# iresearch-toolkit/iresearch

Measured on AMD Instinct MI355X. Metric: queries/sec BM25 top-1000, OR-8-terms, 10M-doc Zipfian index @1/2/4/8 GPU, higher is better.
Workload: dtype u32+f32

## Files before the change

### include/irs_hip.h

```cpp
#ifndef IRS_HIP_H
#define IRS_HIP_H

#include <stddef.h>
#include <stdint.h>

#ifdef __cplusplus
extern "C" {
#endif

#define IRS_HIP_ABI_VERSION 12
#define IRS_HIP_BLOCK_SIZE 128u
#define IRS_HIP_MAX_TERMS 16u
#define IRS_HIP_MAX_K 4096u
#define IRS_HIP_MAX_PHRASE_TERMS 8u
#define IRS_HIP_MAX_PHRASE_ENTRIES 16u
#define IRS_HIP_MAX_EXCLUDED 16u
#define IRS_HIP_NO_TERM 0xFFFFFFFFu
#define IRS_HIP_POS_OFFSETS 1u
#define IRS_HIP_POS_PAYLOADS 2u
#define IRS_HIP_NORM2 0u
#define IRS_HIP_NORM_LEGACY 1u
#define IRS_HIP_WAND_NONE 0u
#define IRS_HIP_WAND_DIV_NORM 1u
#define IRS_HIP_WAND_MAX_FREQ 2u
// ... 214 lines not shown
int irs_hip_device_download(int32_t device, void* h_dst, const void* d_src, uint64_t bytes);
int irs_hip_device_sync(int32_t device, void* stream);
int irs_hip_device_trim(int32_t device);

int irs_hip_device_set_stream_cache(int32_t device, uint64_t bytes);
typedef struct irs_hip_stream_cache_stats {
  uint64_t bytes_held;
  uint64_t budget;
  uint64_t streams;
  uint64_t hits;
  uint64_t misses;
  uint64_t evictions;
} irs_hip_stream_cache_stats;
int irs_hip_device_stream_cache_stats(int32_t device, irs_hip_stream_cache_stats* out);
int irs_hip_batch_stream_counts(irs_hip_batch* batch, uint32_t* distinct, uint32_t* decoded);
int irs_hip_batch_image_counts(irs_hip_batch* batch, uint32_t* distinct, uint32_t* built);
int irs_hip_batch_rescore_paths(irs_hip_batch* batch, uint32_t paths[3]);
int irs_hip_device_image_count(int32_t device, uint64_t* images);
int irs_hip_join_bound_rule(int32_t kind, float norm_const, float norm_length, uint32_t tf_bound,
                            uint16_t* u, float* scale, float* slack, uint32_t* tile_docs);

typedef struct irs_hip_comm irs_hip_comm;
#define IRS_HIP_COMM_ID_BYTES 128u
int irs_hip_comm_unique_id(uint8_t id[IRS_HIP_COMM_ID_BYTES]);
int irs_hip_comm_init_rank(int32_t device, const uint8_t id[IRS_HIP_COMM_ID_BYTES], int32_t n_ranks,
                           int32_t rank, irs_hip_comm** out);
void irs_hip_comm_destroy(irs_hip_comm* comm);
int irs_hip_comm_library(char* buf, size_t cap);
int irs_hip_topk_allgather(irs_hip_comm* comm, const void* d_send, void* d_recv,
                           uint64_t bytes_per_rank, void* stream);
// ... 12 lines not shown
```

### iresearch_amd/_lib.py

```python
from __future__ import annotations

import ctypes as C

import numpy as np

from . import _build

OK, EINVAL, ECORRUPT, ENOMEM, EHIP, EOVERFLOW, EUNSUPPORTED, EPEER = 0, -1, -2, -3, -4, -5, -6, -7
LAYOUT_SCALAR, LAYOUT_SIMD4 = 0, 1
OP_OR, OP_AND, OP_MINMATCH, OP_PHRASE = 0, 1, 2, 3
SCORE_BM25, SCORE_BM15, SCORE_BM1, SCORE_TFIDF, SCORE_TFIDF_NORM = 0, 1, 2, 3, 4
EXCLUDE = 0x100
PHRASE_ALT = 0x200
GROUP_ALT = PHRASE_ALT
PHRASE_REQUIRED = 0x400
NO_TERM = 0xFFFFFFFF
NO_DOC_SET = 0xFFFFFFFF
PATH_AUTO, PATH_ITEMS, PATH_JOINED = 0, 1, 2
WAND_NONE, WAND_DIV_NORM, WAND_MAX_FREQ, WAND_MIN_NORM = 0, 1, 2, 3
MAX_TERMS, MAX_K, MAX_PHRASE_TERMS, MAX_EXCLUDED = 16, 4096, 8, 16
MAX_PHRASE_ENTRIES = 16
K_PLAN, K_PILOT, K_SCORE, K_SELECT, K_COUNT = 0, 1, 2, 3, 4
KERNEL_NAMES = ("k_plan", "k_pilot", "k_score", "k_select")
KERNEL_NAMES_JOINED = ("k_join", "k_join_pilot", "k_join_score", "k_select")
# ... 51 lines not shown
    "irs_hip_batch_set_async", "irs_hip_batch_set_paired_tiles", "irs_hip_batch_paired_tiles",
    "irs_hip_batch_set_comm",
    "irs_hip_term_blockmax",
    "irs_hip_segment_wand_source",
    "irs_hip_batch_touched", "irs_hip_batch_unit_mask",
    "irs_hip_batch_match_sets", "irs_hip_batch_match_sets_to_device",
    "irs_hip_batch_set_doc_sets", "irs_hip_batch_set_doc_sets_host", "irs_hip_batch_doc_set_stats",
    "irs_hip_comm_unique_id", "irs_hip_comm_init_rank", "irs_hip_comm_destroy",
    "irs_hip_comm_library",
    "irs_hip_topk_allgather", "irs_hip_device_alloc", "irs_hip_device_free",
    "irs_hip_device_upload", "irs_hip_device_download", "irs_hip_device_sync",
    "irs_hip_device_trim",
    "irs_hip_device_set_stream_cache", "irs_hip_device_stream_cache_stats",
    "irs_hip_batch_stream_counts",
    "irs_hip_batch_image_counts", "irs_hip_device_image_count", "irs_hip_join_bound_rule",
    "irs_hip_batch_rescore_paths",
)


def bind(L: C.CDLL) -> C.CDLL:
    vp, u32, u64, i32 = C.c_void_p, C.c_uint32, C.c_uint64, C.c_int32
    P = C.POINTER
    L.irs_hip_abi_version.argtypes, L.irs_hip_abi_version.restype = [], u32
    L.irs_hip_strerror.argtypes, L.irs_hip_strerror.restype = [C.c_int], C.c_char_p
    L.irs_hip_device_arch.argtypes, L.irs_hip_device_arch.restype = [i32, C.c_char_p, C.c_size_t], C.c_int
    L.irs_hip_segment_open.argtypes = [P(SegmentDesc), P(vp)]
    L.irs_hip_segment_open.restype = C.c_int
    L.irs_hip_segment_close.argtypes, L.irs_hip_segment_close.restype = [vp], None
    L.irs_hip_segment_device_bytes.argtypes = [vp]
    L.irs_hip_segment_device_bytes.restype = u64
    L.irs_hip_segment_live_docs.argtypes = [vp]
# ... 75 lines not shown
    L.irs_hip_topk_allgather.restype = C.c_int
    L.irs_hip_device_trim.argtypes, L.irs_hip_device_trim.restype = [i32], C.c_int
    L.irs_hip_device_set_stream_cache.argtypes = [i32, u64]
    L.irs_hip_device_set_stream_cache.restype = C.c_int
    L.irs_hip_device_stream_cache_stats.argtypes = [i32, P(StreamCacheStats)]
    L.irs_hip_device_stream_cache_stats.restype = C.c_int
    L.irs_hip_batch_stream_counts.argtypes = [vp, P(u32), P(u32)]
    L.irs_hip_batch_stream_counts.restype = C.c_int
    L.irs_hip_batch_image_counts.argtypes = [vp, P(u32), P(u32)]
    L.irs_hip_batch_image_counts.restype = C.c_int
    L.irs_hip_device_image_count.argtypes, L.irs_hip_device_image_count.restype = [i32, P(u64)], C.c_int
    L.irs_hip_batch_rescore_paths.argtypes, L.irs_hip_batch_rescore_paths.restype = [vp, P(u32)], C.c_int
    L.irs_hip_join_bound_rule.argtypes = [i32, C.c_float, C.c_float, u32, P(C.c_uint16), P(C.c_float),
                                          P(C.c_float), P(u32)]
    L.irs_hip_join_bound_rule.restype = C.c_int
    return L


_lib = None


def lib() -> C.CDLL:
    global _lib
    if _lib is None:
        try:
            import torch
        except ImportError:
            pass
        _lib = bind(C.CDLL(str(_build.build_hip())))
    return _lib
# ... 6 lines not shown
```

### iresearch_amd/csrc/irs_hip.hip

```cpp
#include "irs_hip.h"

#include <algorithm>
#include <atomic>
#include <chrono>
#include <cmath>
#include <condition_variable>
#include <cstdlib>
#include <cstring>
#include <deque>
#include <functional>
#include <map>
#include <memory>
#include <mutex>
#include <new>
#include <thread>
#include <tuple>
#include <type_traits>
#include <unordered_map>
#include <unordered_set>
#include <vector>

#include "gpu_rt.h"
#include "kernels.h"
#include "phrase.h"
// ... 1698 lines not shown
  return guarded([&] {
    if (slack) *slack = kJoinBoundSlack;
    if (tile_docs) *tile_docs = kJoinBoundTile;
    if (!table_kind(kind)) return int(IRS_HIP_EUNSUPPORTED);
    const float sup = join_bound_sup(kind, norm_const, norm_length, tf_bound);
    if (!(sup > 0.f)) return int(IRS_HIP_EUNSUPPORTED);
    const float U = join_bound_scale(sup);
    if (scale) *scale = U;
    if (u)
      for (uint32_t tf = 0; tf < 256u; ++tf)
        for (uint32_t n = 0; n < 256u; ++n)
          u[tf * 256u + n] = uint16_t(join_bound_u(kind, norm_const, norm_length, U, tf, n));
    return int(IRS_HIP_OK);
  });
}
int irs_hip_device_sync(int32_t device, void* stream) {
  return guarded([&] {
    if (!rt::set_device(device)) return int(IRS_HIP_EHIP);
    return int(rt::sync(static_cast<rt::stream_t>(stream)) ? IRS_HIP_OK : IRS_HIP_EHIP);
  });
}
int irs_hip_comm_unique_id(uint8_t id[IRS_HIP_COMM_ID_BYTES]) {
  return guarded([&]() -> int {
    if (!id) return IRS_HIP_EINVAL;
    return rt::comm::unique_id(id) ? IRS_HIP_OK : IRS_HIP_EHIP;
  });
}
int irs_hip_comm_init_rank(int32_t device, const uint8_t id[IRS_HIP_COMM_ID_BYTES], int32_t n_ranks,
                           int32_t rank, irs_hip_comm** out) {
  return guarded([&] { return comm_init_rank_impl(device, id, n_ranks, rank, out); });
// ... 100 lines not shown
```

### iresearch_amd/csrc/join.h

```cpp
#pragma once
#include "score.h"

namespace irs_hip {

constexpr uint32_t kJoinTile = 12288;
constexpr uint32_t kJoinTfMax = 255;
constexpr uint32_t kJoinBlocks = 64;
constexpr uint32_t kJoinChunkTiles = 64;
constexpr uint32_t kJoinChunkPlain = 32;
constexpr uint32_t kJoinCands = 256;
constexpr uint32_t kJoinSlack = 1024;
constexpr uint32_t kJoinQueues = 8;
constexpr uint32_t kAblShift = 0;
constexpr uint32_t kAblCount = 0;
constexpr uint32_t kAblEpi = 0;
constexpr uint32_t kAblNoAdd = 0;
constexpr uint32_t kAblNoTab = 0;
constexpr uint32_t kAblWait = 0;
constexpr uint32_t kAblNoBar = 0;
constexpr uint32_t kJoinCountMask = 15u;
constexpr uint32_t kJoinCountTerms = 15u;
constexpr float kJoinCountRound = 8.f;

enum : uint32_t {
// ... 251 lines not shown
  }
  if (!(sup > 0.f) || !(sup <= 3.0e38f)) return 0.f;
  if (!sqrt_kind(kind) && sup < kJoinBoundSupMin) return 0.f;
  return sup;
}
__host__ __device__ inline float join_bound_scale(float sup) { return (65535.f - 64.f) / sup; }
__host__ __device__ inline uint32_t join_bound_u(int32_t kind, float nc, float nl, float U,
                                                 uint32_t tf, uint32_t norm) {
  const float tref = table_entry(kind, nc, nl, tf ? tf : 1u, norm);
  const float tb = tref + tref * (1.f / 524288.f) + (sqrt_kind(kind) ? 0.f : (1.f / 1048576.f));
  const float r = tb * U + 1.25f;
  const uint32_t u = r >= 65535.f ? 65535u : static_cast<uint32_t>(r);
  return u;
}

struct alignas(16) BoundWg {
  uint64_t src, src_bounds;
  uint64_t dst, dst_bounds;
  uint32_t first;
  uint32_t n;
  uint32_t n_src_tiles, n_dst_tiles;
  int32_t kind;
  float nc, nl;
  float U;
};
static_assert(sizeof(BoundWg) == 64, "BoundWg");

__global__ void __launch_bounds__(kThreads)
k_join_bound(const BoundWg* wgs) {
  const BoundWg W = wgs[blockIdx.x];
  const uint32_t* src = reinterpret_cast<const uint32_t*>(W.src);
  const uint32_t* sb = reinterpret_cast<const uint32_t*>(W.src_bounds);
  uint32_t* dst = reinterpret_cast<uint32_t*>(W.dst);
  uint32_t* db = reinterpret_cast<uint32_t*>(W.dst_bounds);
  if (!W.n) {
    for (uint32_t u = threadIdx.x; u <= W.n_dst_tiles; u += blockDim.x) db[u] = 0u;
    return;
  }
  auto tile_of = [&](uint32_t i, uint32_t lo) {
    uint32_t hi = W.n_src_tiles;
    while (hi - lo > 1u) {
      const uint32_t mid = (lo + hi) >> 1;
      if (sb[mid] <= i) lo = mid; else hi = mid;
    }
    return lo;
  };
  uint32_t t = 0;
  const uint32_t end = W.first + kJoinBoundPerWg < W.n ? W.first + kJoinBoundPerWg : W.n;
  for (uint32_t i = W.first + threadIdx.x; i < end; i += blockDim.x) {
    t = tile_of(i, t);
    const uint32_t e = src[i];
    const uint32_t doc = t * kJoinTile + (e >> 18);
    const uint32_t bt = doc / kJoinBoundTile;
    const uint32_t off = doc - bt * kJoinBoundTile;
    const uint32_t u = join_bound_u(W.kind, W.nc, W.nl, W.U, join_tf(e), (e >> 2) & 255u);
    dst[i] = (off << 18) | u;
    int32_t tp = -1;
    if (i) {
      const uint32_t pt = sb[t] < i ? t : tile_of(i - 1u, 0u);
      tp = int32_t((pt * kJoinTile + (src[i - 1u] >> 18)) / kJoinBoundTile);
    }
    for (int32_t v = tp + 1; v <= int32_t(bt); ++v) db[v] = i;
    if (i + 1u == W.n)
      for (uint32_t v = bt + 1u; v <= W.n_dst_tiles; ++v) db[v] = W.n;
  }
}


struct JoinOff {
  static constexpr uint32_t acc = 0;
  static constexpr uint32_t dummy = 4u * kJoinTile;
  static constexpr uint32_t qts = dummy + 256u;
  static constexpr uint32_t jts = qts + uint32_t(sizeof(DevQTerm)) * kMaxTerms;
  static constexpr uint32_t rng = jts + uint32_t(sizeof(JoinTerm)) * kMaxTerms;
  static constexpr uint32_t cum = rng + 4u * (kJoinChunkTiles + 1u) * kMaxTerms;
  static constexpr uint32_t sig = cum + 4u * kJoinChunkTiles * kMaxTerms;
  static constexpr uint32_t cand = sig + 4u * 2u * 16u;
  static constexpr uint32_t vars = cand + 8u * 2u * kJoinCands;
  static constexpr uint32_t caches = vars + 64u;
// ... 25 lines not shown
};

struct JoinLane {
  uint32_t ent_lo, ent_hi;
  float cs;
  uint32_t mode;
};

enum : int { kJTable = 0, kJRcp = 1, kJSqrt = 2 };
__device__ __forceinline__ int join_form(uint32_t mode) {
  return !(mode & kJoinGeneral) ? kJTable : ((mode & kJoinSqrt) ? kJSqrt : kJRcp);
}
__device__ __forceinline__ uint32_t join_dummy(unsigned lane) {
  return (JoinOff::dummy + 4u * lane) << 16;
}
__device__ __forceinline__ uint32_t join_dummy_img(unsigned lane) {
  return (JoinOffH::dummy + 4u * lane) << 16;
}

template<int FORM, int N, bool COUNT>
__device__ __forceinline__ void join_post(const unsigned char* lds, const uint32_t (&e)[4],
                                          float cs, uint32_t tabofs) {
  float t[N];
  uint32_t fx[N];
#pragma unroll
  for (int k = 0; k < N; ++k) {
    const uint32_t at = (FORM == kJTable) ? ((e[k] & 0xFFFFu) | tabofs) : ((e[k] & 0x3FCu) | tabofs);
    t[k] = kAblNoTab ? __uint_as_float(at | 0x3F000000u) : wave::lds_f32(lds, JoinOff::caches + at);
  }
#pragma unroll
  for (int k = 0; k < N; ++k) wave::keep_f(t[k]);
#pragma unroll
  for (int k = 0; k < N; ++k) {
// ... 85 lines not shown
  float cs;
  uint32_t mode;
  uint32_t e[4];
};

template<int M>
__device__ __forceinline__ void join_begin(JoinRun& r, const JoinLane& T, uint32_t a, uint32_t n,
                                           uint32_t c, uint32_t wv, uint32_t nw_log2,
                                           uint64_t safe, unsigned lane) {
  const uint32_t N = wave::read_lane(c, ((M & kJHalf) ? 2u * kMaxTerms : kMaxTerms) - 1u);
  const uint32_t lo = (N * wv) >> nw_log2, hi = (N * (wv + 1u)) >> nw_log2;
  const uint32_t first = c - n;
  const uint32_t st = lo > first ? lo : first;
  const uint32_t en = hi < c ? hi : c;
  r.cnt = en > st ? en - st : 0u;
  const uint64_t addr = ((uint64_t(T.ent_hi) << 32) | T.ent_lo) + 4ull * (uint64_t(a) + (st - first));
  r.a_lo = uint32_t(addr);
  r.a_hi = uint32_t(addr >> 32);
  uint64_t mask = wave::ballot(r.cnt != 0u);
  uint64_t base = safe;
  uint32_t take = 0;
  r.left = 0;
  r.rest = 0;
  r.cs = 0.f;
  r.mode = 0;
  if (mask) {
    const uint32_t j = uint32_t(__builtin_ctzll(mask));
    mask &= mask - 1ull;
    base = (uint64_t(wave::read_lane(r.a_hi, j)) << 32) | wave::read_lane(r.a_lo, j);
    const uint32_t cnt = wave::read_lane(r.cnt, j);
    r.cs = wave::read_lane_f(T.cs, j);
    if ((M & kJSimple) && (M & kJHalf)) r.mode = j >= kMaxTerms ? uint32_t(kJoinHiHalf) : 0u;
    else if (!(M & kJSimple)) r.mode = wave::read_lane(T.mode, j);
    take = cnt < kJoinPre ? cnt : kJoinPre;
    r.left = cnt - take;
    r.rest = base + 4ull * take;
  }
  r.pre = take;
  r.mask = mask;
  const uint32_t last = take ? (take - 1u) * 4u : 0u;
#pragma unroll
  for (int k = 0; k < 4; ++k) {
    const uint32_t off = lane * 4u + 256u * uint32_t(k);
    r.e[k] = wave::gload_u32(base, off < last ? off : last);
  }
}

template<int M>
__device__ __forceinline__ void join_some(const unsigned char* lds, uint64_t base, uint32_t cnt,
                                          float cs, uint32_t mode, unsigned lane) {
  static_assert((M & kJHalf) == 0, "paired tiles: join_finish_pairs");
  constexpr bool COUNT = (M & kJCount) != 0;
  if (M & kJSimple) {
    join_run<kJTable, COUNT>(lds, base, cnt, cs, 0u, lane);
// ... 25 lines not shown
    for (int k = 0; k < 4; ++k) e[k] = lane + 64u * uint32_t(k) < pre ? r.e[k] : dummy;
    join_post_any<M>(lds, e, (pre + 63u) >> 6, cs0, mode0);
  }
  const uint32_t left = wave::uniform(r.left);
  if (left) join_some<M>(lds, wave::uniform64(r.rest), left, cs0, mode0, lane);
  uint64_t mask = wave::uniform64(r.mask);
  while (mask) {
    const uint32_t j = uint32_t(__builtin_ctzll(mask));
    mask &= mask - 1ull;
    const uint64_t base = (uint64_t(wave::read_lane(r.a_hi, j)) << 32) | wave::read_lane(r.a_lo, j);
    const uint32_t mode = SIMPLE ? 0u : wave::read_lane(T.mode, j);
    join_some<M>(lds, base, wave::read_lane(r.cnt, j), wave::read_lane_f(T.cs, j), mode, lane);
  }
}

struct JoinGroup {
  uint64_t base;
  uint32_t n;
  float cs;
  uint32_t mode;
};
struct JoinSeq {
  uint64_t rest;
  uint32_t left;
  uint64_t mask;
  float cs;
  uint32_t mode;
};
template<int M>
__device__ __forceinline__ bool join_next(JoinSeq& s, const JoinRun& r, const JoinLane& T,
                                          uint64_t safe, JoinGroup& g) {
  bool more = true;
  if (!s.left) {
    if (s.mask) {
      const uint32_t j = uint32_t(__builtin_ctzll(s.mask));
      s.mask &= s.mask - 1ull;
      s.rest = (uint64_t(wave::read_lane(r.a_hi, j)) << 32) | wave::read_lane(r.a_lo, j);
      s.left = wave::read_lane(r.cnt, j);
      s.cs = wave::read_lane_f(T.cs, j);
      s.mode = (M & kJSimple) ? (j >= kMaxTerms ? uint32_t(kJoinHiHalf) : 0u) : wave::read_lane(T.mode, j);
    } else {
      more = false;
    }
  }
  const uint32_t n = s.left < kJoinPre ? s.left : kJoinPre;
  g.base = more ? s.rest : safe;
  g.n = more ? n : 1u;
  g.cs = s.cs;
  g.mode = s.mode;
  s.rest += 4ull * n;
  s.left -= n;
  return more;
}
__device__ __forceinline__ void join_request(const JoinGroup& g, unsigned lane, uint32_t (&x)[4]) {
  const uint32_t last = (g.n - 1u) * 4u;
#pragma unroll
  for (int k = 0; k < 4; ++k) {
    const uint32_t off = lane * 4u + 256u * uint32_t(k);
    x[k] = wave::gload_u32(g.base, off < last ? off : last);
  }
}
template<int N>
__device__ __forceinline__ void join_post_img(const unsigned char* lds, const uint32_t (&e)[4],
                                              float ks, uint32_t sh) {
  uint32_t fx[N];
#pragma unroll
  for (int k = 0; k < N; ++k)
    fx[k] = static_cast<uint32_t>(wave::fma(ks, static_cast<float>(e[k] & 0xFFFFu), 2.f)) << sh;
#pragma unroll
  for (int k = 0; k < N; ++k) {
    if (kAblNoAdd) wave::keep(fx[k]);
    else wave::lds_add(lds, JoinOffH::acc + (e[k] >> 16), fx[k]);
  }
}
__device__ __forceinline__ void join_group_img(const unsigned char* lds, const uint32_t (&x)[4],
                                               const JoinGroup& g, unsigned lane) {
  const uint32_t sh = join_half_shift(g.mode);
  if (g.n == kJoinPre) {
    join_post_img<4>(lds, x, g.cs, sh);
    return;
  }
  const uint32_t dummy = join_dummy_img(lane);
  uint32_t e[4];
#pragma unroll
  for (int k = 0; k < 4; ++k) e[k] = lane + 64u * uint32_t(k) < g.n ? x[k] : dummy;
  const uint32_t slabs = (g.n + 63u) >> 6;
  if (slabs >= 4u) join_post_img<4>(lds, e, g.cs, sh);
  else if (slabs == 3u) join_post_img<3>(lds, e, g.cs, sh);
  else if (slabs == 2u) join_post_img<2>(lds, e, g.cs, sh);
  else join_post_img<1>(lds, e, g.cs, sh);
}

template<int M>
__device__ __forceinline__ void join_finish_pairs(const unsigned char* lds, JoinRun& r,
                                                  const JoinLane& T, uint64_t safe, unsigned lane) {
  static_assert(M == (kJHalf | kJSimple), "join_finish_pairs: paired tiles on bound images");
  const uint32_t pre = wave::uniform(r.pre);
  if (!pre) {
    if (kAblWait) wave::keep_all(r.e);
    return;
  }
  JoinSeq s;
  s.rest = wave::uniform64(r.rest);
  s.left = wave::uniform(r.left);
  s.mask = wave::uniform64(r.mask);
  s.cs = wave::uniform_f(r.cs);
  s.mode = wave::uniform(r.mode);
  JoinGroup ga, gb;
  ga.base = 0;
  ga.n = pre;
  ga.cs = s.cs;
  ga.mode = s.mode;
  uint32_t a[4], b[4];
#pragma unroll
  for (int k = 0; k < 4; ++k) a[k] = r.e[k];
  bool more;
  do {
    const bool second = join_next<M>(s, r, T, safe, gb);
    join_request(gb, lane, b);
    join_group_img(lds, a, ga, lane);
    more = join_next<M>(s, r, T, safe, ga);
    join_request(ga, lane, a);
    if (second) join_group_img(lds, b, gb, lane);
  } while (more);
}

__device__ __forceinline__ void join_prologue(unsigned char* smem, const DevQuery& qd,
                                              const DevQTerm* qterms, const JoinTerm* jterms) {
  DevQTerm* qts = reinterpret_cast<DevQTerm*>(smem + JoinOff::qts);
  JoinQuad* jts = reinterpret_cast<JoinQuad*>(smem + JoinOff::jts);
  uint32_t* sig = reinterpret_cast<uint32_t*>(smem + JoinOff::sig);
  const uint32_t tid = threadIdx.x;
  if (tid < qd.n_terms) {
    const DevQTerm qt = qterms[qd.first_term + tid];
    qts[tid] = qt;
    if (qt.cache_id < kMaxCaches) {
      sig[16u + 1u + 3u * qt.cache_id] = uint32_t(qt.kind);
      sig[16u + 2u + 3u * qt.cache_id] = __float_as_uint(qt.norm_const);
// ... 380 lines not shown
      wave::lds_take4(smem, JoinOff::acc + i * 4u, v0);
      four(i, v0);
    }
    if (!kAblNoBar) __syncthreads();
  };
  for (uint32_t u = 0; u < ntile; u += 2u) {
    join_finish<M>(smem, r0, T, lane);
    begin(u + 2u, r0);
    end_tile(u);
    join_finish<M>(smem, r1, T, lane);
    begin(u + 3u, r1);
    if (u + 1u < ntile) end_tile(u + 1u);
  }
}

__host__ __device__ __forceinline__ uint32_t join_half_slack(uint32_t m) { return 2u * m + 2u; }
static_assert(kJoinBoundSlack * 0.51f + kMaxTerms * (1.f / 128.f + 65.f / 32768.f) < 2.f, "join_half_slack");
template<int M>
__device__ __forceinline__ void join_pairs(unsigned char* smem, const JoinTileCtx& ctx,
                                           const JoinLane& T, uint32_t tile0, uint32_t ntile,
                                           uint32_t wv, uint32_t nw_log2, uint32_t& my_hits) {
  static_assert(M == (kJHalf | kJSimple), "join_pairs: plain disjunctions on bound images");
  const uint32_t* rng = reinterpret_cast<const uint32_t*>(smem + JoinOffH::rng);
  const uint32_t* cum = reinterpret_cast<const uint32_t*>(smem + JoinOffH::cum);
  const uint32_t tid = threadIdx.x;
  const unsigned lane = tid & 63u;
  const uint64_t safe = reinterpret_cast<uint64_t>(ctx.args->jterms);
  const uint32_t npair = (ntile + 1u) >> 1;
  auto begin = [&](uint32_t p, JoinRun& r) {
    uint32_t a = 0, n = 0, c = 0;
    if (lane < 2u * kMaxTerms && p < npair) {
      const uint32_t i = 2u * p + (lane >> 4), j = lane & (kMaxTerms - 1u);
// ... 130 lines not shown
    const uint32_t tile0 = (local / n_units) * per_chunk;
    const DevQuery qd = args->queries[q];
    const uint32_t n_tiles = !HALF ? qd.n_tiles : (qd.n_terms ? args->jterms[qd.first_term].pad[0] : 0u);
    const uint32_t ntile = tile0 >= n_tiles ? 0u
                           : ((n_tiles - tile0) < per_chunk ? (n_tiles - tile0) : per_chunk);
    const uint32_t bs = args->bstar[q];
    uint32_t my_hits = 0;
    uint64_t* lc = lcand + parity * kJoinCands;
    uint32_t* ncand = vars + kJNc + parity;
    if (ntile) {
      for (uint32_t e = tid; e < (ntile + 1u) * kMaxTerms; e += blockDim.x) {
        const uint32_t i = e / kMaxTerms, j = e % kMaxTerms;
        uint32_t v = 0;
        if (j < qd.n_terms)
          v = reinterpret_cast<const uint32_t*>(args->jterms[qd.first_term + j].bounds)[tile0 + i];
        rng[e] = v;
      }
      if constexpr (HALF) {
        JoinQuad* jts = reinterpret_cast<JoinQuad*>(smem + JoinOffH::jts);
        if (tid < kJoinTermQuads * kMaxTerms) {
          const uint32_t j = tid / kJoinTermQuads;
          uint32_t x = 0, y = 0, z = 0, w = 0;
          if (j < qd.n_terms) {
            const uint32_t* src = reinterpret_cast<const uint32_t*>(args->jterms + qd.first_term) + 4u * tid;
            x = src[0]; y = src[1]; z = src[2]; w = src[3];
          }
          jts[tid].x = x; jts[tid].y = y; jts[tid].z = z; jts[tid].w = w;
        }
        __syncthreads();
      } else {
        join_prologue(smem, qd, args->qterms, args->jterms);
// ... 323 lines not shown
```

### iresearch_amd/csrc/plan_join.h

```cpp
#pragma once

namespace {

bool join_allowed(const irs_hip_batch* b) {
  if (b->path_pref == IRS_HIP_PATH_ITEMS) return false;
  if (b->knobs.join_off && b->path_pref != IRS_HIP_PATH_JOINED) return false;
  return !b->phrase && b->acc32;
}
int64_t join_and_saving(const irs_hip_batch* b, const DevQuery& dq) {
  const irs_hip_segment* sg = b->segs[dq.seg];
  uint64_t sum = 0, lead = ~0ull;
  for (uint32_t j = 0; j < dq.n_terms; ++j) {
    const uint64_t df = sg->terms[b->qterms[dq.first_term + j].term].docs_count;
    sum += df;
    lead = std::min(lead, df);
  }
  const uint64_t tiles = sg->dev.num_docs / kJoinTile + 1;
  const uint64_t lead_blocks = lead / kBlock + 1;
  return int64_t(lead_blocks * (2300ull + 400ull * dq.n_terms)) -
         int64_t(4200ull * tiles + (3ull * sum) / 2);
}
constexpr int64_t kJoinAndLaunchCost = 500000000;
int join_and_forced(const irs_hip_batch* b) {
  if (b->path_pref == IRS_HIP_PATH_JOINED) return 1;
// ... 317 lines not shown
  }
  for (irs_hip_segment* sg : b->segs)
    if (prepare_posting_norms(sg) != IRS_HIP_OK) return false;
  lap("  streams: bound images");
  std::vector<BoundWg> bwgs;
  std::vector<JoinTerm> jimgs;
  b->join.img_on = false;
  b->join.img_n_max = 0;
  b->join.n_images = b->join.n_img_private = b->join.n_img_fill = 0;
  b->join.n_bwgs = b->join.n_bwgs_fill = 0;
  if (join_half_ok(b)) {
    std::vector<uint8_t> want(streams.size(), 0), iwhere(streams.size(), kPrivate);
    std::vector<float> img_U(streams.size(), 0.f);
    std::vector<uint64_t> img_ent(streams.size(), 0), img_bnd(streams.size(), 0);
    std::vector<uint32_t> img_tiles(streams.size(), 0), imgs;
    std::vector<std::vector<float>> sup_of(sigs.size(), std::vector<float>(kJoinTfMax + 1u, -1.f));
    bool all = true;
    for (uint32_t u : b->join.units) {
      const DevQuery& dq = b->queries[u];
      if (query_need(dq.op) > 1u) continue;
      if (!b->segs[dq.seg]->dev.has_freq) all = false;
      b->join.img_n_max = std::max(b->join.img_n_max,
                                   (b->segs[dq.seg]->dev.num_docs + kJoinBoundTile - 1) / kJoinBoundTile);
      for (uint32_t j = 0; j < dq.n_terms && all; ++j) {
        const uint32_t si = stream_of[dq.first_term + j];
        if (want[si]) continue;
        want[si] = 1;
        imgs.push_back(si);
        const Sig& sig = sigs[stream_sig[si]];
        const uint32_t tfb = sqrt_kind(sig.kind)
// ... 40 lines not shown
            sl->last_use = ++c.clock;
            if (seen.insert(sl).second) {
              ++sl->pins;
              for (const scache::SlabPtr& sp : c.slabs)
                if (sp.get() == sl) b->join.pinned.push_back(sp);
            }
          }
        }
        std::stable_sort(missed.begin(), missed.end(),
                         [&](uint32_t x, uint32_t y) { return streams[x].seg < streams[y].seg; });
        for (size_t from = 0; from < missed.size();) {
          size_t to = from;
          uint64_t e = 0, bn = 0;
          std::vector<uint64_t> e_off, b_off;
          while (to < missed.size() && streams[missed[to]].seg == streams[missed[from]].seg &&
                 (to == from || e + streams[missed[to]].n <= scache::kSlabEntries)) {
            e_off.push_back(e);
            b_off.push_back(bn);
            e += (uint64_t(streams[missed[to]].n) + scache::kAlign - 1) / scache::kAlign * scache::kAlign;
            bn += uint64_t(img_tiles[missed[to]]) + 1;
            ++to;
          }
          const uint64_t bytes = pool::size_class((e + kJoinSlack + bn) * 4);
          bool room = false;
          {
            std::lock_guard<std::mutex> lock(c.m);
            room = bytes <= budget && scache::make_room_locked(c, bytes, budget, gone);
            if (room) c.held += bytes;
          }
          gone.clear();
          scache::SlabPtr sl;
          if (room) {
            sl = std::make_shared<scache::Slab>();
            if (!sl->mem.alloc((e + kJoinSlack + bn) * 4)) {
              std::lock_guard<std::mutex> lock(c.m);
// ... 21 lines not shown
                sl->images.push_back(k);
            }
            c.slabs.push_back(sl);
            b->join.pinned.push_back(sl);
            b->join.fills.push_back(sl);
          }
          from = to;
        }
        b->join.fill_pending = !b->join.fills.empty();
      }
      uint64_t ie = 0, ib = 0;
      for (uint32_t si : imgs) {
        if (iwhere[si] != kPrivate) continue;
        img_ent[si] = ie;
        img_bnd[si] = ib;
        ie += (uint64_t(streams[si].n) + scache::kAlign - 1) / scache::kAlign * scache::kAlign;
        ib += uint64_t(img_tiles[si]) + 1;
      }
      if (ie + ib) {
        if (!b->join.d_img_entries.alloc((ie + kJoinSlack) * 4) || !b->join.d_img_bounds.alloc((ib + 1) * 4))
          return false;
      } else {
        b->join.d_img_entries.release();
        b->join.d_img_bounds.release();
      }
      for (uint32_t pass = 0; pass < 2; ++pass) {
        for (uint32_t si : imgs) {
          if (iwhere[si] != (pass ? kFill : kPrivate)) continue;
          if (!pass) {
            img_ent[si] = reinterpret_cast<uint64_t>(b->join.d_img_entries.as<uint32_t>() + img_ent[si]);
            img_bnd[si] = reinterpret_cast<uint64_t>(b->join.d_img_bounds.as<uint32_t>() + img_bnd[si]);
          }
// ... 17 lines not shown
            ++(pass ? b->join.n_bwgs_fill : b->join.n_bwgs);
          }
        }
      }
      if (bwgs.size() > 0x7FFFFFFFull) return false;
      b->join.n_images = uint32_t(imgs.size());
      jimgs.assign(b->qterms.size(), JoinTerm{});
      for (uint32_t u : b->join.units) {
        const DevQuery& dq = b->queries[u];
        if (query_need(dq.op) > 1u) continue;
        for (uint32_t j = 0; j < dq.n_terms; ++j) {
          const uint32_t si = stream_of[dq.first_term + j];
          JoinTerm& ji = jimgs[dq.first_term + j];
          ji.entries = img_ent[si];
          ji.bounds = img_bnd[si];
          ji.cs = (b->qterms[dq.first_term + j].c0 * dq.fx_mul) * (1.f / 32768.f) / img_U[si];
          ji.mode = 0;
          ji.pad[0] = img_tiles[si];
          ji.pad[1] = 0;
        }
      }
      b->join.img_on = true;
    }
  }
  if (b->join.img_on) {
    if (!b->join.d_jimgs.alloc(jimgs.size() * sizeof(JoinTerm)) ||
        !b->join.d_bwgs.alloc(std::max<size_t>(1, bwgs.size()) * sizeof(BoundWg)) ||
        !b->up.copy(b->join.d_jimgs.p, jimgs.data(), jimgs.size() * sizeof(JoinTerm)) ||
        (!bwgs.empty() && !b->up.copy(b->join.d_bwgs.p, bwgs.data(), bwgs.size() * sizeof(BoundWg))))
      return false;
  }
  lap("  streams: k_join records");
  JoinWg* wg_recs = static_cast<JoinWg*>(b->up.put(b->join.d_wgs.p, wgs.size() * sizeof(JoinWg)));
  if (!wg_recs && !wgs.empty()) return false;
  for (size_t i = 0; i < wgs.size(); ++i) {
    const StreamRec& sr = streams[wgs[i].stream];
    const irs_hip_segment* sg = b->segs[sr.seg];
    const DevSegment& ds = sg->dev;
    const DevTerm& t = sg->terms[sr.term];
    JoinWg& w = wg_recs[i];
    w.entries = sr.entries;
// ... 57 lines not shown
  b->join.images_built_last = b->join.img_on ? b->join.n_img_private + (fill ? b->join.n_img_fill : 0u) : 0u;
  if (!grid && !bgrid) return true;
  bool ok = true;
  if (fill)
    for (const scache::SlabPtr& s : b->join.fills)
      ok = ok && rt::dmemset(s->mem.as<uint32_t>() + s->entries, 0, kJoinSlack * 4, st);
  if (!ok) return false;
  if (grid)
    with_layout(b->seg->dev.layout, [&](auto L) {
      RT_LAUNCH((k_join<decltype(L)::value>), grid, kThreads, 0, st, b->join.d_wgs.as<JoinWg>());
    });
  ok = rt::last_error_ok();
  if (ok && bgrid) {
    ok = wait_for_streams(b, st);
    if (ok) {
      RT_LAUNCH(k_join_bound, bgrid, kThreads, 0, st, b->join.d_bwgs.as<BoundWg>());
      ok = rt::last_error_ok();
    }
  }
  if (ok && fill) {
    for (const scache::SlabPtr& s : b->join.fills) {
      s->fill_stream = st;
      ok = ok && s->filled.record(st);
    }
    if (ok) {
      scache::Cache& c = scache::of(b->seg->device);
      std::lock_guard<std::mutex> lock(c.m);
      for (const scache::SlabPtr& s : b->join.fills) s->queued = true;
      b->join.fill_pending = false;
    }
  }
  return ok;
// ... 192 lines not shown
```

### iresearch_amd/search.py

```python
from __future__ import annotations

import ctypes as C
import math
from dataclasses import dataclass, field, replace

import numpy as np

from . import _lib
from ._lib import (EXCLUDE, HIT, NO_TERM, OP_AND, OP_MINMATCH, OP_OR, OP_PHRASE, PHRASE_ALT, PHRASE_REQUIRED, QUERY, SCORE_BM1, SCORE_BM15, SCORE_BM25,
                   SCORE_TFIDF, SCORE_TFIDF_NORM, TERM_META, TERM_SCORER, SegmentDesc)

f32 = np.float32



@dataclass(frozen=True)
class TermStats:
    idf: np.float32
    norm_const: np.float32 = f32(0)
    norm_length: np.float32 = f32(0)


class BM25:

# ... 857 lines not shown


def join_bound_rule(kind, norm_const, norm_length, tf_bound, L=None):
    L = L or _lib.lib()
    u = np.zeros((256, 256), np.uint16)
    scale, slack, tile = C.c_float(), C.c_float(), C.c_uint32()
    rc = L.irs_hip_join_bound_rule(kind, norm_const, norm_length, tf_bound,
                                   u.ctypes.data_as(C.POINTER(C.c_uint16)), C.byref(scale),
                                   C.byref(slack), C.byref(tile))
    if rc == _lib.EUNSUPPORTED:
        return None
    _lib.check(L, rc, "irs_hip_join_bound_rule")
    return u, float(scale.value), float(slack.value), int(tile.value)


def set_stream_cache(nbytes, L=None, device=0):
    L = L or _lib.lib()
    _lib.check(L, L.irs_hip_device_set_stream_cache(device, int(nbytes)),
               "irs_hip_device_set_stream_cache")



@dataclass
class SegmentStats:
    docs_with_field: int
    total_term_freq: int
    docs_count: np.ndarray


def prepare(filters, scorer, segment_stats, required_terms=False):
# ... 432 lines not shown
```

Measured before the change: 243,100.

## Pad join image tiles to 64-entry slabs and use integer half-word scoring

Image entries for each bound tile are now padded to a multiple of 64 with dummy entries, so the half-precision join path can load whole slabs without per-lane masking. Bound building is split into a tile-offset/prefix-scan kernel and a scatter kernel. The float FMA plus shift is replaced by a 16-bit integer multiply-add and byte permute with a precomputed integer scale. The intent is to cut per-group branching and ALU work in the hot accumulate loop. The costs are larger image memory from padding, an extra kernel launch, and a changed quantization slack.

```diff
diff --git a/include/irs_hip.h b/include/irs_hip.h
--- a/include/irs_hip.h
+++ b/include/irs_hip.h
@@ -252,6 +252,9 @@
 } irs_hip_stream_cache_stats;
 int irs_hip_device_stream_cache_stats(int32_t device, irs_hip_stream_cache_stats* out);
 int irs_hip_batch_stream_counts(irs_hip_batch* batch, uint32_t* distinct, uint32_t* decoded);
+int irs_hip_join_half_rule(float cs, float scale, uint32_t* k);
+int irs_hip_join_half_probe(int32_t device, const uint32_t* entries, uint32_t n, uint32_t k,
+                            uint32_t high_half, uint32_t* out);
 int irs_hip_batch_image_counts(irs_hip_batch* batch, uint32_t* distinct, uint32_t* built);
 int irs_hip_batch_rescore_paths(irs_hip_batch* batch, uint32_t paths[3]);
 int irs_hip_device_image_count(int32_t device, uint64_t* images);
diff --git a/iresearch_amd/_lib.py b/iresearch_amd/_lib.py
--- a/iresearch_amd/_lib.py
+++ b/iresearch_amd/_lib.py
@@ -89,7 +89,7 @@
     "irs_hip_device_set_stream_cache", "irs_hip_device_stream_cache_stats",
     "irs_hip_batch_stream_counts",
     "irs_hip_batch_image_counts", "irs_hip_device_image_count", "irs_hip_join_bound_rule",
-    "irs_hip_batch_rescore_paths",
+    "irs_hip_batch_rescore_paths", "irs_hip_join_half_rule", "irs_hip_join_half_probe",
 )
 
 
@@ -195,6 +195,9 @@
     L.irs_hip_join_bound_rule.argtypes = [i32, C.c_float, C.c_float, u32, P(C.c_uint16), P(C.c_float),
                                           P(C.c_float), P(u32)]
     L.irs_hip_join_bound_rule.restype = C.c_int
+    L.irs_hip_join_half_rule.argtypes, L.irs_hip_join_half_rule.restype = [C.c_float, C.c_float, P(u32)], C.c_int
+    L.irs_hip_join_half_probe.argtypes = [i32, P(u32), u32, u32, u32, P(u32)]
+    L.irs_hip_join_half_probe.restype = C.c_int
     return L
 
 
diff --git a/iresearch_amd/csrc/irs_hip.hip b/iresearch_amd/csrc/irs_hip.hip
--- a/iresearch_amd/csrc/irs_hip.hip
+++ b/iresearch_amd/csrc/irs_hip.hip
@@ -1736,6 +1736,29 @@
     return int(IRS_HIP_OK);
   });
 }
+int irs_hip_join_half_rule(float cs, float scale, uint32_t* k) {
+  return guarded([&] {
+    if (!k || !(cs >= 0.f) || !(scale > 0.f)) return int(IRS_HIP_EINVAL);
+    *k = join_half_k(cs, scale);
+    return int(IRS_HIP_OK);
+  });
+}
+int irs_hip_join_half_probe(int32_t device, const uint32_t* entries, uint32_t n, uint32_t k,
+                            uint32_t high_half, uint32_t* out) {
+  return guarded([&] {
+    if (!entries || !out || !n || !k || k > 65535u) return int(IRS_HIP_EINVAL);
+    if (device < 0 || device >= rt::device_count() || !rt::set_device(device)) return int(IRS_HIP_EHIP);
+    uint32_t* d = static_cast<uint32_t*>(rt::dmalloc(size_t(n) * 8));
+    if (!d) return int(IRS_HIP_ENOMEM);
+    bool ok = rt::h2d(d, entries, size_t(n) * 4, nullptr) && rt::sync(nullptr);
+    if (ok) {
+      RT_LAUNCH(k_join_half_probe, 1, kThreads, 0, nullptr, d, n, k, high_half, d + n);
+      ok = rt::last_error_ok() && rt::d2h(out, d + n, size_t(n) * 4, nullptr) && rt::sync(nullptr);
+    }
+    rt::dfree(d);
+    return int(ok ? IRS_HIP_OK : IRS_HIP_EHIP);
+  });
+}
 int irs_hip_device_sync(int32_t device, void* stream) {
   return guarded([&] {
     if (!rt::set_device(device)) return int(IRS_HIP_EHIP);
diff --git a/iresearch_amd/csrc/join.h b/iresearch_amd/csrc/join.h
--- a/iresearch_amd/csrc/join.h
+++ b/iresearch_amd/csrc/join.h
@@ -289,6 +289,11 @@
   return u;
 }
 
+__host__ __device__ inline uint64_t join_image_entries(uint64_t n, uint64_t tiles) {
+  return n + 63u * (n < tiles ? n : tiles);
+}
+constexpr uint32_t kJoinSlab = 64;
+
 struct alignas(16) BoundWg {
   uint64_t src, src_bounds;
   uint64_t dst, dst_bounds;
@@ -302,16 +307,57 @@
 static_assert(sizeof(BoundWg) == 64, "BoundWg");
 
 __global__ void __launch_bounds__(kThreads)
+k_join_bound_tiles(const BoundWg* wgs) {
+  const BoundWg W = wgs[blockIdx.x];
+  if (W.first) return;
+  const uint32_t* src = reinterpret_cast<const uint32_t*>(W.src);
+  const uint32_t* sb = reinterpret_cast<const uint32_t*>(W.src_bounds);
+  uint32_t* db = reinterpret_cast<uint32_t*>(W.dst_bounds);
+  uint32_t* raw = db + W.n_dst_tiles + 1u;
+  __shared__ uint32_t part[kThreads / 64u];
+  __shared__ uint32_t carry;
+  const uint32_t tid = threadIdx.x;
+  for (uint32_t v = tid; v <= W.n_dst_tiles; v += blockDim.x) {
+    const uint64_t doc = uint64_t(v) * kJoinBoundTile;
+    const uint64_t t = doc / kJoinTile;
+    uint32_t lo = W.n;
+    if (W.n && t < W.n_src_tiles) {
+      const uint32_t want = uint32_t(doc - t * kJoinTile);
+      uint32_t hi = sb[t + 1u];
+      lo = sb[t];
+      while (lo < hi) {
+        const uint32_t mid = lo + ((hi - lo) >> 1);
+        if ((src[mid] >> 18) < want) lo = mid + 1u; else hi = mid;
+      }
+    }
+    raw[v] = lo;
+  }
+  if (tid == 0) carry = 0u;
+  __syncthreads();
+  for (uint32_t v0 = 0; v0 <= W.n_dst_tiles; v0 += blockDim.x) {
+    const uint32_t v = v0 + tid;
+    uint32_t c = 0;
+    if (v < W.n_dst_tiles) c = (raw[v + 1u] - raw[v] + kJoinSlab - 1u) & ~(kJoinSlab - 1u);
+    const uint32_t inc = wave::inclusive_scan(c);
+    if ((tid & 63u) == 63u) part[tid >> 6] = inc;
+    __syncthreads();
+    uint32_t before = carry;
+    for (uint32_t w = 0; w < (tid >> 6); ++w) before += part[w];
+    if (v <= W.n_dst_tiles) db[v] = before + inc - c;
+    __syncthreads();
+    if (tid == blockDim.x - 1u) carry = before + inc;
+    __syncthreads();
+  }
+}
+__global__ void __launch_bounds__(kThreads)
 k_join_bound(const BoundWg* wgs) {
   const BoundWg W = wgs[blockIdx.x];
+  if (!W.n) return;
   const uint32_t* src = reinterpret_cast<const uint32_t*>(W.src);
   const uint32_t* sb = reinterpret_cast<const uint32_t*>(W.src_bounds);
   uint32_t* dst = reinterpret_cast<uint32_t*>(W.dst);
-  uint32_t* db = reinterpret_cast<uint32_t*>(W.dst_bounds);
-  if (!W.n) {
-    for (uint32_t u = threadIdx.x; u <= W.n_dst_tiles; u += blockDim.x) db[u] = 0u;
-    return;
-  }
+  const uint32_t* db = reinterpret_cast<const uint32_t*>(W.dst_bounds);
+  const uint32_t* raw = db + W.n_dst_tiles + 1u;
   auto tile_of = [&](uint32_t i, uint32_t lo) {
     uint32_t hi = W.n_src_tiles;
     while (hi - lo > 1u) {
@@ -327,17 +373,16 @@
     const uint32_t e = src[i];
     const uint32_t doc = t * kJoinTile + (e >> 18);
     const uint32_t bt = doc / kJoinBoundTile;
+    if (bt >= W.n_dst_tiles) continue;
     const uint32_t off = doc - bt * kJoinBoundTile;
     const uint32_t u = join_bound_u(W.kind, W.nc, W.nl, W.U, join_tf(e), (e >> 2) & 255u);
-    dst[i] = (off << 18) | u;
-    int32_t tp = -1;
-    if (i) {
-      const uint32_t pt = sb[t] < i ? t : tile_of(i - 1u, 0u);
-      tp = int32_t((pt * kJoinTile + (src[i - 1u] >> 18)) / kJoinBoundTile);
-    }
-    for (int32_t v = tp + 1; v <= int32_t(bt); ++v) db[v] = i;
-    if (i + 1u == W.n)
-      for (uint32_t v = bt + 1u; v <= W.n_dst_tiles; ++v) db[v] = W.n;
+    const uint32_t r0 = raw[bt], r1 = raw[bt + 1u];
+    if (i < r0 || i >= r1) continue;
+    const uint32_t at = db[bt] + (i - r0);
+    dst[at] = (off << 18) | u;
+    if (i + 1u == r1)
+      for (uint32_t p = at + 1u, pe = db[bt + 1u]; p < pe; ++p)
+        dst[p] = (4u * kJoinBoundTile + 4u * (p & (kJoinSlab - 1u))) << 16;
   }
 }
 
@@ -393,9 +438,6 @@
 __device__ __forceinline__ uint32_t join_dummy(unsigned lane) {
   return (JoinOff::dummy + 4u * lane) << 16;
 }
-__device__ __forceinline__ uint32_t join_dummy_img(unsigned lane) {
-  return (JoinOffH::dummy + 4u * lane) << 16;
-}
 
 template<int FORM, int N, bool COUNT>
 __device__ __forceinline__ void join_post(const unsigned char* lds, const uint32_t (&e)[4],
@@ -511,7 +553,9 @@
   const uint32_t st = lo > first ? lo : first;
   const uint32_t en = hi < c ? hi : c;
   r.cnt = en > st ? en - st : 0u;
-  const uint64_t addr = ((uint64_t(T.ent_hi) << 32) | T.ent_lo) + 4ull * (uint64_t(a) + (st - first));
+  constexpr uint32_t kUnit = (M & kJHalf) ? 4u * kJoinSlab : 4u;
+  constexpr uint32_t kPre = (M & kJHalf) ? kJoinPre / kJoinSlab : kJoinPre;
+  const uint64_t addr = ((uint64_t(T.ent_hi) << 32) | T.ent_lo) + uint64_t(kUnit) * (uint64_t(a) + (st - first));
   r.a_lo = uint32_t(addr);
   r.a_hi = uint32_t(addr >> 32);
   uint64_t mask = wave::ballot(r.cnt != 0u);
@@ -529,12 +573,19 @@
     r.cs = wave::read_lane_f(T.cs, j);
     if ((M & kJSimple) && (M & kJHalf)) r.mode = j >= kMaxTerms ? uint32_t(kJoinHiHalf) : 0u;
     else if (!(M & kJSimple)) r.mode = wave::read_lane(T.mode, j);
-    take = cnt < kJoinPre ? cnt : kJoinPre;
+    take = cnt < kPre ? cnt : kPre;
     r.left = cnt - take;
-    r.rest = base + 4ull * take;
+    r.rest = base + uint64_t(kUnit) * take;
   }
   r.pre = take;
   r.mask = mask;
+  if (M & kJHalf) {
+    const uint32_t top = take ? take - 1u : 0u;
+#pragma unroll
+    for (uint32_t k = 0; k < 4u; ++k)
+      r.e[k] = wave::gload_u32(base, lane * 4u + 256u * (k < top ? k : top));
+    return;
+  }
   const uint32_t last = take ? (take - 1u) * 4u : 0u;
 #pragma unroll
   for (int k = 0; k < 4; ++k) {
@@ -590,6 +641,8 @@
   }
 }
 
+constexpr uint32_t kJoinPreSlabs = kJoinPre / kJoinSlab;
+static_assert(kJoinPreSlabs == 4u, "a group is four loads");
 struct JoinGroup {
   uint64_t base;
   uint32_t n;
@@ -619,52 +672,62 @@
       more = false;
     }
   }
-  const uint32_t n = s.left < kJoinPre ? s.left : kJoinPre;
+  const uint32_t n = s.left < kJoinPreSlabs ? s.left : kJoinPreSlabs;
   g.base = more ? s.rest : safe;
   g.n = more ? n : 1u;
   g.cs = s.cs;
   g.mode = s.mode;
-  s.rest += 4ull * n;
+  s.rest += 256ull * n;
   s.left -= n;
   return more;
 }
 __device__ __forceinline__ void join_request(const JoinGroup& g, unsigned lane, uint32_t (&x)[4]) {
-  const uint32_t last = (g.n - 1u) * 4u;
-#pragma unroll
-  for (int k = 0; k < 4; ++k) {
-    const uint32_t off = lane * 4u + 256u * uint32_t(k);
-    x[k] = wave::gload_u32(g.base, off < last ? off : last);
-  }
+  const uint32_t top = g.n - 1u;
+#pragma unroll
+  for (uint32_t k = 0; k < 4u; ++k)
+    x[k] = wave::gload_u32(g.base, lane * 4u + 256u * (k < top ? k : top));
+}
+__host__ __device__ __forceinline__ uint32_t join_half_sel(uint32_t hi) { return hi ? 0x03020c0cu : 0x0c0c0302u; }
+__device__ __forceinline__ uint32_t join_half_term(uint32_t e, uint32_t k, uint32_t add, uint32_t sel) {
+#if defined(__HIP_DEVICE_COMPILE__)
+  uint32_t p, out;
+  asm("v_mad_u32_u16 %0, %1, %2, %3" : "=v"(p) : "v"(e), "s"(k), "v"(add));
+  asm("v_perm_b32 %0, %1, %1, %2" : "=v"(out) : "v"(p), "s"(sel));
+  return out;
+#else
+  const uint32_t p = (e & 0xFFFFu) * k + add;
+  return sel == join_half_sel(0u) ? p >> 16 : p & 0xFFFF0000u;
+#endif
+}
+__global__ void __launch_bounds__(kThreads)
+k_join_half_probe(const uint32_t* e, uint32_t n, uint32_t k, uint32_t hi, uint32_t* out) {
+  const uint32_t ks = wave::uniform(k), sel = wave::uniform(join_half_sel(hi));
+  uint32_t add = 2u << 16;
+  wave::keep(add);
+  for (uint32_t i = threadIdx.x; i < n; i += blockDim.x) out[i] = join_half_term(e[i], ks, add, sel);
 }
 template<int N>
 __device__ __forceinline__ void join_post_img(const unsigned char* lds, const uint32_t (&e)[4],
-                                              float ks, uint32_t sh) {
+                                              uint32_t k, uint32_t add, uint32_t sel) {
   uint32_t fx[N];
 #pragma unroll
-  for (int k = 0; k < N; ++k)
-    fx[k] = static_cast<uint32_t>(wave::fma(ks, static_cast<float>(e[k] & 0xFFFFu), 2.f)) << sh;
-#pragma unroll
-  for (int k = 0; k < N; ++k) {
-    if (kAblNoAdd) wave::keep(fx[k]);
-    else wave::lds_add(lds, JoinOffH::acc + (e[k] >> 16), fx[k]);
+  for (int i = 0; i < N; ++i) fx[i] = join_half_term(e[i], k, add, sel);
+#pragma unroll
+  for (int i = 0; i < N; ++i) {
+    if (kAblNoAdd) wave::keep(fx[i]);
+    else wave::lds_add(lds, JoinOffH::acc + (e[i] >> 16), fx[i]);
   }
 }
 __device__ __forceinline__ void join_group_img(const unsigned char* lds, const uint32_t (&x)[4],
-                                               const JoinGroup& g, unsigned lane) {
-  const uint32_t sh = join_half_shift(g.mode);
-  if (g.n == kJoinPre) {
-    join_post_img<4>(lds, x, g.cs, sh);
-    return;
-  }
-  const uint32_t dummy = join_dummy_img(lane);
-  uint32_t e[4];
-#pragma unroll
-  for (int k = 0; k < 4; ++k) e[k] = lane + 64u * uint32_t(k) < g.n ? x[k] : dummy;
-  const uint32_t slabs = (g.n + 63u) >> 6;
-  if (slabs >= 4u) join_post_img<4>(lds, e, g.cs, sh);
-  else if (slabs == 3u) join_post_img<3>(lds, e, g.cs, sh);
-  else if (slabs == 2u) join_post_img<2>(lds, e, g.cs, sh);
-  else join_post_img<1>(lds, e, g.cs, sh);
+                                               const JoinGroup& g) {
+  const uint32_t k = __float_as_uint(g.cs);
+  const uint32_t sel = join_half_sel(g.mode & uint32_t(kJoinHiHalf));
+  uint32_t add = 2u << 16;
+  wave::keep(add);
+  if (g.n >= 4u) join_post_img<4>(lds, x, k, add, sel);
+  else if (g.n == 3u) join_post_img<3>(lds, x, k, add, sel);
+  else if (g.n == 2u) join_post_img<2>(lds, x, k, add, sel);
+  else join_post_img<1>(lds, x, k, add, sel);
 }
 
 template<int M>
@@ -694,10 +757,10 @@
   do {
     const bool second = join_next<M>(s, r, T, safe, gb);
     join_request(gb, lane, b);
-    join_group_img(lds, a, ga, lane);
+    join_group_img(lds, a, ga);
     more = join_next<M>(s, r, T, safe, ga);
     join_request(ga, lane, a);
-    if (second) join_group_img(lds, b, gb, lane);
+    if (second) join_group_img(lds, b, gb);
   } while (more);
 }
 
@@ -1108,8 +1171,13 @@
   }
 }
 
-__host__ __device__ __forceinline__ uint32_t join_half_slack(uint32_t m) { return 2u * m + 2u; }
-static_assert(kJoinBoundSlack * 0.51f + kMaxTerms * (1.f / 128.f + 65.f / 32768.f) < 2.f, "join_half_slack");
+__host__ __device__ __forceinline__ uint32_t join_half_slack(uint32_t m) { return 3u * m + 2u; }
+static_assert(kJoinBoundSlack * 0.5005f + kMaxTerms * (65.f / 32768.f) < 2.f, "join_half_slack");
+static_assert(32768u + 3u * kMaxTerms + 2u < 65536u, "a 16-bit sum of kMaxTerms terms");
+inline uint32_t join_half_k(float cs, float U) {
+  const double v = std::ceil(double(cs) / double(U) * 2.0);
+  return v >= 1.0 ? (v < 65535.0 ? uint32_t(v) : 65535u) : 1u;
+}
 template<int M>
 __device__ __forceinline__ void join_pairs(unsigned char* smem, const JoinTileCtx& ctx,
                                            const JoinLane& T, uint32_t tile0, uint32_t ntile,
@@ -1270,7 +1338,7 @@
         uint32_t v = 0;
         if (j < qd.n_terms)
           v = reinterpret_cast<const uint32_t*>(args->jterms[qd.first_term + j].bounds)[tile0 + i];
-        rng[e] = v;
+        rng[e] = HALF ? v / kJoinSlab : v;
       }
       if constexpr (HALF) {
         JoinQuad* jts = reinterpret_cast<JoinQuad*>(smem + JoinOffH::jts);
diff --git a/iresearch_amd/csrc/plan_join.h b/iresearch_amd/csrc/plan_join.h
--- a/iresearch_amd/csrc/plan_join.h
+++ b/iresearch_amd/csrc/plan_join.h
@@ -355,6 +355,11 @@
     std::vector<float> img_U(streams.size(), 0.f);
     std::vector<uint64_t> img_ent(streams.size(), 0), img_bnd(streams.size(), 0);
     std::vector<uint32_t> img_tiles(streams.size(), 0), imgs;
+    auto img_entries = [&](uint32_t si) {
+      return (join_image_entries(streams[si].n, img_tiles[si]) + kJoinSlab - 1) / kJoinSlab * kJoinSlab;
+    };
+    auto img_bounds = [&](uint32_t si) { return 2 * (uint64_t(img_tiles[si]) + 1); };
+    static_assert(kJoinSlab % scache::kAlign == 0, "a slab-aligned image is stream-aligned");
     std::vector<std::vector<float>> sup_of(sigs.size(), std::vector<float>(kJoinTfMax + 1u, -1.f));
     bool all = true;
     for (uint32_t u : b->join.units) {
@@ -425,11 +430,11 @@
           uint64_t e = 0, bn = 0;
           std::vector<uint64_t> e_off, b_off;
           while (to < missed.size() && streams[missed[to]].seg == streams[missed[from]].seg &&
-                 (to == from || e + streams[missed[to]].n <= scache::kSlabEntries)) {
+                 (to == from || e + img_entries(missed[to]) <= scache::kSlabEntries)) {
             e_off.push_back(e);
             b_off.push_back(bn);
-            e += (uint64_t(streams[missed[to]].n) + scache::kAlign - 1) / scache::kAlign * scache::kAlign;
-            bn += uint64_t(img_tiles[missed[to]]) + 1;
+            e += img_entries(missed[to]);
+            bn += img_bounds(missed[to]);
             ++to;
           }
           const uint64_t bytes = pool::size_class((e + kJoinSlack + bn) * 4);
@@ -481,8 +486,8 @@
         if (iwhere[si] != kPrivate) continue;
         img_ent[si] = ie;
         img_bnd[si] = ib;
-        ie += (uint64_t(streams[si].n) + scache::kAlign - 1) / scache::kAlign * scache::kAlign;
-        ib += uint64_t(img_tiles[si]) + 1;
+        ie += img_entries(si);
+        ib += img_bounds(si);
       }
       if (ie + ib) {
         if (!b->join.d_img_entries.alloc((ie + kJoinSlack) * 4) || !b->join.d_img_bounds.alloc((ib + 1) * 4))
@@ -530,7 +535,8 @@
           JoinTerm& ji = jimgs[dq.first_term + j];
           ji.entries = img_ent[si];
           ji.bounds = img_bnd[si];
-          ji.cs = (b->qterms[dq.first_term + j].c0 * dq.fx_mul) * (1.f / 32768.f) / img_U[si];
+          const uint32_t k16 = join_half_k(b->qterms[dq.first_term + j].c0 * dq.fx_mul, img_U[si]);
+          std::memcpy(&ji.cs, &k16, 4);
           ji.mode = 0;
           ji.pad[0] = img_tiles[si];
           ji.pad[1] = 0;
@@ -540,7 +546,7 @@
     }
   }
   if (b->join.img_on) {
-    if (!b->join.d_jimgs.alloc(jimgs.size() * sizeof(JoinTerm)) ||
+    if (!b->join.d_jimgs.alloc(std::max<size_t>(1024, jimgs.size() * sizeof(JoinTerm))) ||
         !b->join.d_bwgs.alloc(std::max<size_t>(1, bwgs.size()) * sizeof(BoundWg)) ||
         !b->up.copy(b->join.d_jimgs.p, jimgs.data(), jimgs.size() * sizeof(JoinTerm)) ||
         (!bwgs.empty() && !b->up.copy(b->join.d_bwgs.p, bwgs.data(), bwgs.size() * sizeof(BoundWg))))
@@ -628,8 +634,12 @@
   if (ok && bgrid) {
     ok = wait_for_streams(b, st);
     if (ok) {
-      RT_LAUNCH(k_join_bound, bgrid, kThreads, 0, st, b->join.d_bwgs.as<BoundWg>());
+      RT_LAUNCH(k_join_bound_tiles, bgrid, kThreads, 0, st, b->join.d_bwgs.as<BoundWg>());
       ok = rt::last_error_ok();
+      if (ok) {
+        RT_LAUNCH(k_join_bound, bgrid, kThreads, 0, st, b->join.d_bwgs.as<BoundWg>());
+        ok = rt::last_error_ok();
+      }
     }
   }
   if (ok && fill) {
diff --git a/iresearch_amd/search.py b/iresearch_amd/search.py
--- a/iresearch_amd/search.py
+++ b/iresearch_amd/search.py
@@ -895,6 +895,23 @@
     return u, float(scale.value), float(slack.value), int(tile.value)
 
 
+def join_half_rule(cs, scale, L=None):
+    L = L or _lib.lib()
+    k = C.c_uint32()
+    _lib.check(L, L.irs_hip_join_half_rule(cs, scale, C.byref(k)), "irs_hip_join_half_rule")
+    return int(k.value)
+
+
+def join_half_probe(entries, k, high_half, L=None, device=0):
+    L = L or _lib.lib()
+    e = np.ascontiguousarray(entries, np.uint32)
+    out = np.zeros(e.size, np.uint32)
+    p = C.POINTER(C.c_uint32)
+    _lib.check(L, L.irs_hip_join_half_probe(device, e.ctypes.data_as(p), e.size, int(k), int(bool(high_half)),
+                                            out.ctypes.data_as(p)), "irs_hip_join_half_probe")
+    return out
+
+
 def set_stream_cache(nbytes, L=None, device=0):
     L = L or _lib.lib()
     _lib.check(L, L.irs_hip_device_set_stream_cache(device, int(nbytes)),
```

Result: faster. 251,500 (median of 6 runs) (+3.4%).
